# ViV99/slam-experiments

Measured on NVIDIA B200. Metric: hamming_pairs_per_sec, higher is better.
Workload: dtype u8

## Files before the change

### slam_experiments_b200/csrc/hm_tc.cu

```cuda
#include <math.h>
#include <stdlib.h>

#include <mutex>
#include <type_traits>

#include <cuda_fp16.h>

#include "hm_common.cuh"
#include "hm_tcgen05.cuh"

#ifndef HM_F4_TILE_N
#define HM_F4_TILE_N 128
#endif

namespace hm {

namespace {

constexpr int kRowBlock = 128;
constexpr int kMBlocks = 2;
constexpr int kBlockM = kRowBlock * kMBlocks;
constexpr int kSlabBytes = kRowBlock * 128;
constexpr int kPadRows = HM_PREPARED_TILE_ROWS;
constexpr int kTmemCols = 512;
constexpr uint32_t kSpinLimit = 1u << 26;

static_assert(kPadRows % kBlockM == 0, "prepared padding must cover whole query blocks");

struct CoreI8 {
    using Acc = int;
    static constexpr int kSlabs = 2;
    static constexpr int kRowBytes = HM_PREPARED_ROW_BYTES;
    static constexpr int kTileN = 128;
    static constexpr int kStages = 4;
    static constexpr int kUnits = 4;
    static constexpr int kColSplit = 1;
    static constexpr bool kRegisterHandover = false;
    static constexpr bool kScales = false;
    static constexpr int kPrologueTiles = 45;
    static __device__ __forceinline__ Acc lowest() { return INT_MIN; }
    static __device__ __forceinline__ Acc from_bits(uint32_t x) { return (int)x; }
    static __device__ __forceinline__ Acc max3(Acc a, Acc b, Acc c) { return __vimax3_s32(a, b, c); }
    static __device__ __forceinline__ Acc max2(Acc a, Acc b) { return max(a, b); }
    static __device__ __forceinline__ bool valid(Acc v) { return v >= -256; }
    static __device__ __forceinline__ unsigned distance(Acc v) { return (unsigned)((256 - v) >> 1); }
    static __device__ __forceinline__ unsigned encode(Acc v) { return (unsigned)(v + 257); }
    static __device__ __forceinline__ Acc floor_from(unsigned e) { return (int)e - 259; }
    static __device__ __forceinline__ uint32_t pack2(uint32_t lo, uint32_t hi) { return ((uint32_t)max((int)lo, -32768) & 0xFFFFu) | ((uint32_t)max((int)hi, -32768) << 16); }
    static __device__ __forceinline__ Acc unpack(uint32_t p, int hi) { return hi ? (int)p >> 16 : (int)(short)(p & 0xFFFFu); }
    static constexpr uint32_t kLowestBits = 0x80000000u;
};

struct CoreF4 {
    using Acc = float;
    static constexpr int kSlabs = 1;
    static constexpr int kRowBytes = HM_PREPARED_F4_ROW_BYTES;
    static constexpr int kTileN = HM_F4_TILE_N;
#ifndef HM_F4_STAGES
#define HM_F4_STAGES 6
#endif
    static constexpr int kStages = HM_F4_TILE_N == 96 ? 10 : HM_F4_TILE_N == 64 ? 14 : HM_F4_STAGES;
#ifndef HM_F4_UNITS
#define HM_F4_UNITS (HM_F4_TILE_N == 96 ? 5 : HM_F4_TILE_N == 64 ? 7 : 3)
#endif
    static constexpr int kUnits = HM_F4_UNITS;
    static constexpr int kColSplit = 2;
    static constexpr bool kRegisterHandover = true;
    static constexpr bool kScales = true;
    static constexpr int kPrologueTiles = 90;
    static __device__ __forceinline__ Acc lowest() { return -INFINITY; }
    static __device__ __forceinline__ Acc from_bits(uint32_t x) { return __uint_as_float(x); }
    static __device__ __forceinline__ Acc max3(Acc a, Acc b, Acc c) { return fmaxf(fmaxf(a, b), c); }
    static __device__ __forceinline__ Acc max2(Acc a, Acc b) { return fmaxf(a, b); }
    static __device__ __forceinline__ bool valid(Acc v) { return v >= -256.0f; }
    static __device__ __forceinline__ unsigned distance(Acc v) { return (unsigned)((256 - (int)v) >> 1); }
    static __device__ __forceinline__ unsigned encode(Acc v) { return (unsigned)((int)v + 257); }
    static __device__ __forceinline__ Acc floor_from(unsigned e) { return (float)((int)e - 259); }
    static __device__ __forceinline__ uint32_t pack2(uint32_t lo, uint32_t hi)
    {
        const __half2 h = __floats2half2_rn(__uint_as_float(lo), __uint_as_float(hi));
        return *reinterpret_cast<const uint32_t*>(&h);
    }
    static __device__ __forceinline__ Acc unpack(uint32_t p, int hi)
    {
        const __half2 h = *reinterpret_cast<const __half2*>(&p);
        return hi ? __high2float(h) : __low2float(h);
    }
    static constexpr uint32_t kLowestBits = 0xFF800000u;
};

template <class C> __host__ __device__ constexpr int row_block_bytes() { return kRowBlock * C::kRowBytes; }
template <class C> __host__ __device__ constexpr int a_bytes() { return kMBlocks * row_block_bytes<C>(); }
template <class C> __host__ __device__ constexpr int b_stage_bytes() { return C::kTileN * C::kRowBytes; }
template <class C> __host__ __device__ constexpr int epilogue_warps() { return 4 * kMBlocks * C::kColSplit; }
template <class C> __host__ __device__ constexpr int control_warps() { return C::kRegisterHandover ? 4 : 2; }
template <class C> __host__ __device__ constexpr int threads() { return 32 * (control_warps<C>() + epilogue_warps<C>()); }
constexpr int kHandoverBytes = kBlockM * 16;
constexpr int kBarrierBytes = 512;
template <class C> __host__ __device__ constexpr int smem_bytes() { return 1024 + a_bytes<C>() + C::kStages * b_stage_bytes<C>() + kBarrierBytes + kHandoverBytes; }
static_assert((2 * CoreF4::kStages + 1 + 2 * CoreF4::kUnits) * 8 + 16 <= kBarrierBytes, "barrier block");
static_assert((2 * CoreI8::kStages + 1 + 2 * CoreI8::kUnits) * 8 + 16 <= kBarrierBytes, "barrier block");
__host__ __device__ constexpr int ct_gcd(int a, int b) { return b == 0 ? a : ct_gcd(b, a % b); }
template <class C> __host__ __device__ constexpr int issuer_period() { return C::kStages / ct_gcd(C::kStages, C::kUnits) * C::kUnits; }
constexpr int kScaleCols = 32;
constexpr int kScaleCol = kTmemCols - kScaleCols;
static_assert(CoreF4::kUnits * CoreF4::kTileN <= kScaleCol, "accumulator units must end before the scale factors");

struct PrepareParams {
    const uint8_t* bits;
    long long n, stride, batch_stride;
    long long padded_rows;
    uint8_t* out;
};

__global__ void __launch_bounds__(256) hm_prepare_kernel(const PrepareParams P)
{
    const long long chunks_per_problem = P.padded_rows * 16;
    const long long o = (long long)blockIdx.x * blockDim.x + threadIdx.x;
    if (o >= chunks_per_problem) return;
    const int b = blockIdx.y;
    const long long rb = o >> 11;
    const int rem = (int)(o & 2047);
    const int slab = rem >> 10;
    const int rem2 = rem & 1023;
    const int rr = (rem2 >> 3) & 7;
    const int r = ((rem2 >> 6) << 3) | rr;
    const int c = (rem2 & 7) ^ rr;
    const long long row = rb * kRowBlock + r;
    uint4 v = make_uint4(0, 0, 0, 0);
    if (row < P.n) {
        const uint8_t* src = P.bits + (long long)b * P.batch_stride + row * P.stride + slab * 16 + c * 2;
        const unsigned bits16 = (unsigned)src[0] | ((unsigned)src[1] << 8);
        unsigned w[4];
#pragma unroll
        for (int i = 0; i < 4; ++i) {
            const unsigned nib = (bits16 >> (4 * i)) & 0xF;
            const unsigned spread = (nib & 1) | ((nib & 2) << 7) | ((nib & 4) << 14) | ((nib & 8) << 21);
            w[i] = (spread * 0xFEu) ^ 0xFFFFFFFFu;
        }
        v = make_uint4(w[0], w[1], w[2], w[3]);
    }
    uint4* dst = reinterpret_cast<uint4*>(P.out + (long long)b * P.padded_rows * HM_PREPARED_ROW_BYTES);
    dst[o] = v;
}

__device__ __forceinline__ uint4 expand_bits_e2m1(unsigned bits32)
{
    unsigned w[4];
#pragma unroll
    for (int i = 0; i < 4; ++i) {
        const unsigned by = (bits32 >> (8 * i)) & 0xFF;
        unsigned sgn = 0;
#pragma unroll
        for (int j = 0; j < 8; ++j) sgn |= ((by >> j) & 1u) << (4 * j + 3);
        w[i] = 0xAAAAAAAAu ^ sgn;
    }
    return make_uint4(w[0], w[1], w[2], w[3]);
}

__global__ void __launch_bounds__(256) hm_prepare_f4_kernel(const PrepareParams P)
{
    const long long chunks_per_problem = P.padded_rows * 8;
    const long long o = (long long)blockIdx.x * blockDim.x + threadIdx.x;
    if (o >= chunks_per_problem) return;
    const int b = blockIdx.y;
    const long long rb = o >> 10;
    const int rem = (int)(o & 1023);
    const int rr = (rem >> 3) & 7;
    const int r = ((rem >> 6) << 3) | rr;
    const int c = (rem & 7) ^ rr;
    const long long row = rb * kRowBlock + r;
    uint4 v = make_uint4(0, 0, 0, 0);
    if (row < P.n) {
        const unsigned bits32 = *reinterpret_cast<const unsigned*>(P.bits + (long long)b * P.batch_stride + row * P.stride + c * 4);
        v = expand_bits_e2m1(bits32);
    }
    uint4* dst = reinterpret_cast<uint4*>(P.out + (long long)b * P.padded_rows * HM_PREPARED_F4_ROW_BYTES);
    dst[o] = v;
}

struct TcParams {
    const uint8_t* qbits;
// ... 104 lines not shown
__device__ __forceinline__ void tmem_ld_fence4(uint32_t (&a)[32], uint32_t (&b)[32], uint32_t (&c)[32], uint32_t (&d)[32])
{
    asm volatile("tcgen05.wait::ld.sync.aligned;\n" : HM_R32(a), HM_R32(b), HM_R32(c), HM_R32(d) : : "memory");
}
__device__ __forceinline__ void tmem_ld_fence48(uint32_t (&a)[32], uint32_t (&b)[16])
{
    asm volatile("tcgen05.wait::ld.sync.aligned;\n" : HM_R32(a), HM_R8(b, 0), HM_R8(b, 8) : : "memory");
}
__device__ __forceinline__ void tmem_ld_fence64(uint32_t (&a)[64])
{
    asm volatile("tcgen05.wait::ld.sync.aligned;\n" : HM_R8(a, 0), HM_R8(a, 8), HM_R8(a, 16), HM_R8(a, 24), HM_R8(a, 32), HM_R8(a, 40), HM_R8(a, 48), HM_R8(a, 56) : : "memory");
}

template <class C, int kMode, int kGroups = 4>
__device__ __forceinline__ void scan_chunk(const uint32_t* r, unsigned colbase, Top2<typename C::Acc>& s)
{
    using Acc = typename C::Acc;
    static_assert(kGroups == 2 || kGroups == 4 || kGroups == 8, "8-column groups per compare");
    Acc gm[kGroups];
#pragma unroll
    for (int g = 0; g < kGroups; ++g) {
        const int o = g * 8;
        gm[g] = C::max3(C::max3(C::from_bits(r[o]), C::from_bits(r[o + 1]), C::from_bits(r[o + 2])),
                        C::max3(C::from_bits(r[o + 3]), C::from_bits(r[o + 4]), C::from_bits(r[o + 5])),
                        C::max2(C::from_bits(r[o + 6]), C::from_bits(r[o + 7])));
    }
    Acc m;
    if constexpr (kGroups == 8) m = C::max3(C::max3(gm[0], gm[1], gm[2]), C::max3(gm[3], gm[4], gm[5]), C::max2(gm[6], gm[7]));
    else if constexpr (kGroups == 4) m = C::max3(gm[0], gm[1], C::max2(gm[2], gm[3]));
    else m = C::max2(gm[0], gm[1]);
    constexpr bool kFloor = kMode == 1, kTop1 = kMode == 2;
    if (m > (kFloor ? s.f : kTop1 ? s.v1 : s.v2)) {
#if HM_TC_TRACE
        s.slow += 1;
#endif
#pragma unroll
        for (int g = 0; g < kGroups; ++g) {
            const Acc x = gm[g];
            if (x > (kFloor ? s.f : kTop1 ? s.v1 : s.v2)) {
                const int o = g * 8;
                const uint32_t p0 = C::pack2(r[o], r[o + 1]), p1 = C::pack2(r[o + 2], r[o + 3]);
                const uint32_t p2 = C::pack2(r[o + 4], r[o + 5]), p3 = C::pack2(r[o + 6], r[o + 7]);
                const unsigned idx = colbase + o;
                if (kTop1 || x > s.v1) {
                    if (!kTop1) {
                        s.v2 = s.v1; s.i2 = s.i1;
                        s.sb[0] = s.sa[0]; s.sb[1] = s.sa[1]; s.sb[2] = s.sa[2]; s.sb[3] = s.sa[3];
                    }
                    s.v1 = x; s.i1 = idx;
                    s.sa[0] = p0; s.sa[1] = p1; s.sa[2] = p2; s.sa[3] = p3;
                } else {
                    s.v2 = x; s.i2 = idx;
                    s.sb[0] = p0; s.sb[1] = p1; s.sb[2] = p2; s.sb[3] = p3;
                }
                if (kFloor) s.f = C::max2(s.v2, s.f);
            }
        }
    }
}

template <class C, int kN>
__device__ __forceinline__ void mask_tail(uint32_t* r, unsigned colbase, unsigned limit)
{
    if (colbase + kN > limit) {
#pragma unroll
        for (int j = 0; j < kN; ++j)
            if (colbase + j >= limit) r[j] = C::kLowestBits;
    }
}

#ifndef HM_ARRIVE_ELECT
#define HM_ARRIVE_ELECT 1
#endif
#ifndef HM_SCAN_FLAT64
#define HM_SCAN_FLAT64 1
#endif
#ifndef HM_FLOOR_DENSE_TILES
#define HM_FLOOR_DENSE_TILES 32
#endif
#ifndef HM_FLOOR_LATE_MASK
#define HM_FLOOR_LATE_MASK 15
#endif

#ifndef HM_F4_A_TMEM
#define HM_F4_A_TMEM 0
#endif
constexpr int kATmemCol = 384;
constexpr int kATmemColsPerBlock = 32;

template <class C>
__device__ __forceinline__ void issue_half(int h, uint32_t a_block, uint32_t b_stage, uint32_t tmem_d, uint32_t idesc,
                                           uint32_t tmem_sf)
{
    constexpr int kHalf = C::kSlabs * 2;
#pragma unroll
    for (int jj = 0; jj < kHalf; ++jj) {
        const int j = h * kHalf + jj;
        const int slab = j >> 2, k = j & 3;
        const uint64_t db = ptx::kmajor_sw128_desc_from_lo(b_stage + ((slab * kSlabBytes + k * 32) >> 4));
        if constexpr (C::kScales && HM_F4_A_TMEM) {
            ptx::mma_mxf4_ts(tmem_d, a_block + 8 * j, db, idesc, tmem_sf, tmem_sf + kScaleCols / 2, j != 0);
        } else {
            const uint64_t da = ptx::kmajor_sw128_desc_from_lo(a_block + ((slab * kSlabBytes + k * 32) >> 4));
            if constexpr (C::kScales) ptx::mma_mxf4_ss(tmem_d, da, db, idesc, tmem_sf, tmem_sf + kScaleCols / 2, j != 0);
            else                      ptx::mma_i8_ss(tmem_d, da, db, idesc, j != 0);
        }
    }
}

template <class C, int kMode>
__device__ __forceinline__ void tc_knn2_body(const TcParams& P)
{
    constexpr bool kFloor = kMode == 1;
    using Acc = typename C::Acc;
    constexpr int kStages = C::kStages;
    constexpr int kUnits = C::kUnits;
    constexpr int kABytes = a_bytes<C>();
    constexpr int kBStageBytes = b_stage_bytes<C>();
    constexpr int kRowBlockBytes = row_block_bytes<C>();
    constexpr int kTileN = C::kTileN;

    extern __shared__ uint8_t smem_raw[];
    uint8_t* smem = smem_raw + ((1024u - (ptx::smem_u32(smem_raw) & 1023u)) & 1023u);
    uint8_t* smem_a = smem;
    uint8_t* smem_b = smem + kABytes;
    uint64_t* bars = reinterpret_cast<uint64_t*>(smem + kABytes + kStages * kBStageBytes);
    uint64_t* full_bar = bars;
    uint64_t* empty_bar = bars + kStages;
    uint64_t* a_full_bar = bars + 2 * kStages;
    uint64_t* tmem_full_bar = bars + 2 * kStages + 1;
    uint64_t* tmem_empty_bar = tmem_full_bar + kUnits;
    uint32_t* tmem_base_slot = reinterpret_cast<uint32_t*>(tmem_empty_bar + kUnits);
    uint32_t* smem_base_slot = tmem_base_slot + 2;
    ulonglong2* handover = reinterpret_cast<ulonglong2*>(smem + kABytes + kStages * kBStageBytes + kBarrierBytes);

    const int warp = __shfl_sync(0xffffffffu, threadIdx.x >> 5, 0);
    const int lane = threadIdx.x & 31;
    if (threadIdx.x == 0) cta_mark(P, 0);
    if (threadIdx.x == 0 && (blockIdx.x | blockIdx.y | blockIdx.z) == 0 && P.clock_probe) {
        unsigned long long t;
        asm volatile("mov.u64 %0, %%globaltimer;" : "=l"(t));
        P.clock_probe[0] = (long long)t;
        P.clock_probe[1] = clock64();
    }
    const int qb = blockIdx.x;
    const int split = blockIdx.y;
    const int b = blockIdx.z;

    const uint32_t cs = ptx::cluster_nctarank();
    const uint32_t crank = ptx::cluster_ctarank();
    const uint16_t cmask = (uint16_t)((1u << cs) - 1);
    const bool has_a = qb < P.q_blocks_valid;
    auto rows_present = [&]() -> long long { return P.nq_dyn ? min((long long)__ldg(P.nq_dyn + b), P.nq) : P.nq; };
    if (P.nq_dyn && (long long)(qb - (int)crank) * kBlockM >= rows_present()) return;

    const int tile_begin = split * P.tiles_per_split;
    const int tile_end = min(tile_begin + P.tiles_per_split, P.ntiles);
    const int my_tiles = tile_end - tile_begin;

    constexpr int kProducerWarp = kIssuerLast ? epilogue_warps<C>() : 0;
    constexpr int kIssuerWarp = kIssuerLast ? epilogue_warps<C>() + 1 : 1;
    constexpr int kFirstEpiWarp = kIssuerLast ? 0 : 2;
    static_assert(kIssuerLast || !C::kRegisterHandover, "the control warps must form the last warpgroup");
    static_assert(!C::kRegisterHandover || (epilogue_warps<C>() == 16 && threads<C>() == 640),
                  "the register budget (4 x 32 + 16 x 112 = 20 x 96) assumes 20 warps launched at 96 registers");
    if (warp == kProducerWarp && lane == 0) {
        *smem_base_slot = ptx::smem_u32(smem);
        for (int i = 0; i < kStages; ++i) {
            ptx::mbar_init(&full_bar[i], 1);
            ptx::mbar_init(&empty_bar[i], cs);
        }
        ptx::mbar_init(a_full_bar, 1);
        for (int i = 0; i < kUnits; ++i) {
            ptx::mbar_init(&tmem_full_bar[i], 1);
            ptx::mbar_init(&tmem_empty_bar[i], 4 * C::kColSplit);
        }
        ptx::fence_barrier_init();
        ptx::fence_proxy_async();
    } else if (warp == kIssuerWarp) {
        ptx::tmem_alloc(tmem_base_slot, kTmemCols);
        ptx::tmem_relinquish();
    }
    ptx::tc_fence_before();
    if (cs > 1) ptx::cluster_sync();
    else __syncthreads();
    ptx::tc_fence_after();
    const uint32_t tmem_base = *tmem_base_slot;

    if constexpr (C::kScales) {
        if (warp >= kFirstEpiWarp && warp < kFirstEpiWarp + 4) {
            uint32_t ones[32];
#pragma unroll
            for (int i = 0; i < 32; ++i) ones[i] = 0x7F7F7F7Fu;
            const uint32_t taddr = tmem_base + ((uint32_t)((warp & 3) * 32) << 16) + kScaleCol;
            static_assert(kScaleCols == 32, "one x32 store per lane quarter");
            ptx::tmem_st_32x32(taddr, ones);
            ptx::tmem_st_wait();
        }
        if (HM_F4_A_TMEM) {
            static_assert(!HM_F4_A_TMEM || C::kUnits * C::kTileN <= kATmemCol, "accumulator units overlap the A operand");
            static_assert(!HM_F4_A_TMEM || kATmemCol + kMBlocks * kATmemColsPerBlock <= kScaleCol, "A operand overlaps the scale factors");
            if (warp >= kFirstEpiWarp && warp < kFirstEpiWarp + 4 * kMBlocks) {
                const int wq = warp & 3, wblk = ((warp - kFirstEpiWarp) >> 2) & 1;
                const int r = wq * 32 + lane;
                const long long qrow = (long long)qb * kBlockM + wblk * kRowBlock + r;
                uint32_t words[32];
#pragma unroll
                for (int i = 0; i < 32; ++i) words[i] = 0u;
                if (qrow < rows_present()) {
                    if (P.qbits) {
                        const int* qidx = P.q_index ? P.q_index + (long long)b * P.q_index_batch_stride : nullptr;
                        const long long srow = qidx ? (long long)__ldg(qidx + qrow) : qrow;
                        const uint4* src = reinterpret_cast<const uint4*>(P.qbits + (long long)b * P.q_bits_batch_stride + srow * P.q_bits_stride);
                        const uint4 lo = src[0], hi = src[1];
                        const unsigned bits[8] = {lo.x, lo.y, lo.z, lo.w, hi.x, hi.y, hi.z, hi.w};
#pragma unroll
                        for (int c = 0; c < 8; ++c) {
                            const uint4 v = expand_bits_e2m1(bits[c]);
                            words[4 * c] = v.x; words[4 * c + 1] = v.y; words[4 * c + 2] = v.z; words[4 * c + 3] = v.w;
                        }
                    } else if (has_a) {
                        const uint8_t* img = P.qprep + ((long long)b * P.q_padded + (long long)qb * kBlockM + wblk * kRowBlock) * C::kRowBytes;
                        const uint4* row = reinterpret_cast<const uint4*>(img + (r >> 3) * 1024 + (r & 7) * 128);
#pragma unroll
                        for (int c = 0; c < 8; ++c) {
                            const uint4 v = row[c ^ (r & 7)];
                            words[4 * c] = v.x; words[4 * c + 1] = v.y; words[4 * c + 2] = v.z; words[4 * c + 3] = v.w;
                        }
                    }
                }
                ptx::tmem_st_32x32(tmem_base + ((uint32_t)(wq * 32) << 16) + kATmemCol + wblk * kATmemColsPerBlock, words);
                ptx::tmem_st_wait();
            }
        } else if (P.qbits) {
            const uint8_t* qsrc = P.qbits + (long long)b * P.q_bits_batch_stride;
            const int* qidx = P.q_index ? P.q_index + (long long)b * P.q_index_batch_stride : nullptr;
            const long long nq_eff = rows_present();
            for (int o = threadIdx.x; o < kBlockM * 8; o += blockDim.x) {
                const int blk = o >> 10, rem = o & 1023;
                const int rr = (rem >> 3) & 7;
                const int r = ((rem >> 6) << 3) | rr;
                const int c = (rem & 7) ^ rr;
                const long long qrow = (long long)qb * kBlockM + blk * kRowBlock + r;
                uint4 v = make_uint4(0, 0, 0, 0);
                if (qrow < nq_eff) {
                    const long long srow = qidx ? (long long)__ldg(qidx + qrow) : qrow;
                    v = expand_bits_e2m1(*reinterpret_cast<const unsigned*>(qsrc + srow * P.q_bits_stride + c * 4));
                }
                reinterpret_cast<uint4*>(smem_a)[o] = v;
            }
            ptx::fence_proxy_async();
        }
        ptx::tc_fence_before();
        __syncthreads();
        ptx::tc_fence_after();
    }

    if (threadIdx.x == 0) cta_mark(P, 1);
    ulonglong2 my_keys = make_ulonglong2(kNoMatch, kNoMatch);
    long long my_row = -1;
    int my_row_in_cta = 0;

    auto run_producer = [&]() {
        if (lane == 0) {
            if (has_a && !P.qbits && !(C::kScales && HM_F4_A_TMEM)) {
                const uint8_t* qsrc = P.qprep + ((long long)b * P.q_padded + (long long)qb * kBlockM) * C::kRowBytes;
                ptx::mbar_arrive_expect_tx(a_full_bar, kABytes);
                ptx::bulk_g2s(smem_a, qsrc, kABytes, a_full_bar);
            }
            const uint8_t* tsrc = P.tprep + (long long)b * P.t_padded * C::kRowBytes;
            const uint32_t piece = kBStageBytes / cs;
            for (int i = 0; i < (HM_TC_EXPERIMENT >= 5 ? 0 : my_tiles); ++i) {
                const int stage = i % kStages;
                const uint32_t use = i / kStages;
#if HM_TC_EXPERIMENT < 4
                bounded_wait(&empty_bar[stage], (use & 1) ^ 1, P.error_flag);
#endif
                trace_mark(P, i, 0);
                ptx::mbar_arrive_expect_tx(&full_bar[stage], kBStageBytes);
                uint8_t* dst = smem_b + stage * kBStageBytes + crank * piece;
                const uint8_t* src = tsrc + (long long)(tile_begin + i) * kBStageBytes + crank * piece;
                if (cs > 1) ptx::bulk_g2s_multicast(dst, src, piece, &full_bar[stage], cmask);
                else        ptx::bulk_g2s(dst, src, piece, &full_bar[stage]);
            }
        }
    };
    auto run_issuer = [&]() {
        const bool leader = ptx::elect_one();
        const uint32_t idesc = C::kScales ? ptx::make_mxf4_idesc(kRowBlock, kTileN) : ptx::make_i8_idesc(kRowBlock, kTileN);
        constexpr bool kATmem = C::kScales && HM_F4_A_TMEM;
        const uint32_t a_addr = kATmem ? tmem_base + kATmemCol : ptx::smem_u32(smem_a) >> 4;
        constexpr uint32_t kABlockStep = kATmem ? (uint32_t)kATmemColsPerBlock : (uint32_t)(kRowBlockBytes >> 4);
        const uint32_t b_addr = ptx::smem_u32(smem_b) >> 4;
        const uint32_t tmem_sf = tmem_base + kScaleCol;
        if (has_a && !P.qbits && !(C::kScales && HM_F4_A_TMEM)) bounded_wait(a_full_bar, 0, P.error_flag);
        constexpr int kPeriod = issuer_period<C>();
        static_assert(kPeriod % kStages == 0 && (2 * kPeriod) % kUnits == 0 && ((2 * kPeriod / kUnits) & 1) == 0,
                      "unit parities must repeat with the period");
        uint32_t sphase = 0;
        bool ready0 = false;
        for (int base = 0; base < my_tiles; base += kPeriod) {
#pragma unroll
            for (int j = 0; j < kPeriod; ++j) {
                if (base + j < my_tiles) {
                    const int stage = j % kStages;
                    const uint32_t full_par = sphase ^ ((j / kStages) & 1);
                    const int unit_a = (2 * j) % kUnits, unit_b = (2 * j + 1) % kUnits;
                    const uint32_t par_a = (((2 * j) / kUnits) & 1) ^ 1, par_b = (((2 * j + 1) / kUnits) & 1) ^ 1;
                    const uint32_t b_stage = b_addr + stage * (kBStageBytes >> 4);
                    if (leader) trace_mark(P, base + j, 7);
                    if (!ready0) {
#if HM_TC_EXPERIMENT < 4
                        bounded_wait(&full_bar[stage], full_par, P.error_flag);
#endif
#if HM_TC_EXPERIMENT < 3
                        bounded_wait(&tmem_empty_bar[unit_a], par_a, P.error_flag);
#endif
                    }
                    if (leader) trace_mark(P, base + j, 1);
                    ptx::tc_fence_after();
                    if (leader) issue_half<C>(0, a_addr, b_stage, tmem_base + unit_a * kTileN, idesc, tmem_sf);
#if HM_TC_EXPERIMENT >= 3
                    const bool ready1 = true;
#else
                    const bool ready1 = __all_sync(0xffffffffu, ptx::mbar_test_wait(&tmem_empty_bar[unit_b], par_b));
#endif
                    if (leader) {
                        issue_half<C>(1, a_addr, b_stage, tmem_base + unit_a * kTileN, idesc, tmem_sf);
#if HM_TC_EXPERIMENT != 6 && HM_COMMIT_MODE == 0
                        ptx::tc_commit(&tmem_full_bar[unit_a]);
#endif
                    }
                    if (!ready1) bounded_wait(&tmem_empty_bar[unit_b], par_b, P.error_flag);
                    if (leader) trace_mark(P, base + j, 6);
                    ptx::tc_fence_after();
                    if (leader) issue_half<C>(0, a_addr + kABlockStep, b_stage, tmem_base + unit_b * kTileN, idesc, tmem_sf);
                    ready0 = false;
                    if (base + j + 1 < my_tiles) {
                        const int n = j + 1;
#if HM_TC_EXPERIMENT >= 4
                        ready0 = true;
#else
                        ready0 = __all_sync(0xffffffffu,
                                            ptx::mbar_test_wait(&full_bar[n % kStages], sphase ^ ((n / kStages) & 1))
#if HM_TC_EXPERIMENT < 3
                                            && ptx::mbar_test_wait(&tmem_empty_bar[(2 * n) % kUnits], (((2 * n) / kUnits) & 1) ^ 1)
#endif
                                            );
#endif
                    }
                    if (leader) {
                        issue_half<C>(1, a_addr + kABlockStep, b_stage, tmem_base + unit_b * kTileN, idesc, tmem_sf);
#if HM_TC_EXPERIMENT == 6 || HM_COMMIT_MODE == 1
                        ptx::tc_commit(&tmem_full_bar[unit_a]);
#endif
                        ptx::tc_commit(&tmem_full_bar[unit_b]);
                        if (cs > 1) ptx::tc_commit_multicast(&empty_bar[stage], cmask);
                        else        ptx::tc_commit(&empty_bar[stage]);
                    }
                }
            }
            sphase ^= (kPeriod / kStages) & 1;
        }
        __syncwarp();
    };
    auto run_epilogue = [&]() {
        constexpr int kCols = kTileN / C::kColSplit;
        const int quarter = warp & 3;
        const int mblk = ((warp - kFirstEpiWarp) >> 2) & 1;
        const int half = (warp - kFirstEpiWarp) >> 3;
        const int row_in_cta = mblk * kRowBlock + quarter * 32 + lane;
        const long long row = (long long)qb * kBlockM + row_in_cta;
        Top2<Acc> s;
        s.v1 = s.v2 = C::lowest();
        s.i1 = s.i2 = 0;
#pragma unroll
        for (int e = 0; e < 4; ++e) s.sa[e] = s.sb[e] = 0;
        s.f = C::floor_from(0);
#if HM_TC_TRACE
        s.slow = 0;
#endif
        unsigned floor_code = 0;
        const long long first_row = (long long)tile_begin * kTileN;
        const unsigned limit = (unsigned)min((long long)my_tiles * kTileN, P.nt - first_row);
        const uint32_t bars_addr = ptx::lds_volatile_u32(ptx::smem_u32(smem_base_slot)) + kABytes + kStages * kBStageBytes;
        const uint32_t unit_full_addr = bars_addr + (2 * kStages + 1) * 8;
        const uint32_t unit_empty_addr = unit_full_addr + kUnits * 8;
        int unit = mblk;
        uint32_t unit_use = 0;
        unsigned floor_pending = 0;
        auto refresh_floor = [&](int i) {
            if constexpr (kFloor) {
                if (i < HM_FLOOR_DENSE_TILES || (i & HM_FLOOR_LATE_MASK) == 0) {
                    floor_code = max(floor_code, floor_pending);
                    s.f = C::max2(s.f, C::floor_from(floor_code));
                    if (row < P.nq) {
                        unsigned* floor_ptr = P.row_floor + ((long long)b * P.nq + row);
                        const unsigned e = C::valid(s.v2) ? C::encode(s.v2) : 0u;
                        if (e > floor_code) { atomicMax(floor_ptr, e); floor_code = e; }
                        floor_pending = __ldcg(floor_ptr);
                    }
                }
            }
        };
        auto process_tile = [&](int i) {
            bounded_wait_addr(unit_full_addr + unit * 8, unit_use & 1, P.error_flag);
#if HM_TC_TRACE == 2
            if (warp == kFirstEpiWarp && lane == 0 && (i == 8 || i == 32 || i == 64 || i == 192)) cta_mark(P, i == 8 ? 5 : i == 32 ? 6 : i == 64 ? 7 : 8);
#endif
            if (warp == kFirstEpiWarp && lane == 0) trace_mark(P, i, 3);
            if (warp == kFirstEpiWarp + 7 && lane == 0) trace_mark(P, i, 5);
            ptx::tc_fence_after();
            const uint32_t taddr = tmem_base + ((uint32_t)(quarter * 32) << 16) + unit * kTileN + half * kCols;
            const unsigned colbase = (unsigned)i * kTileN + half * kCols;
            if constexpr (C::kColSplit == 1) {
                uint32_t r0[32], r1[32], r2[32], r3[32];
                ptx::tmem_ld_32x32(taddr, r0);
                ptx::tmem_ld_32x32(taddr + 32, r1);
                ptx::tmem_ld_32x32(taddr + 64, r2);
                ptx::tmem_ld_32x32(taddr + 96, r3);
                refresh_floor(i);
                tmem_ld_fence4(r0, r1, r2, r3);
                ptx::tc_fence_before();
                __syncwarp();
                if (HM_ARRIVE_ELECT ? ptx::elect_one() : lane == 0) ptx::mbar_arrive_addr(unit_empty_addr + unit * 8);
                if (colbase + kCols > limit) {
                    mask_tail<C, 32>(r0, colbase, limit);
                    mask_tail<C, 32>(r1, colbase + 32, limit);
                    mask_tail<C, 32>(r2, colbase + 64, limit);
                    mask_tail<C, 32>(r3, colbase + 96, limit);
                }
                scan_chunk<C, kMode>(r0, colbase, s);
                scan_chunk<C, kMode>(r1, colbase + 32, s);
                scan_chunk<C, kMode>(r2, colbase + 64, s);
                scan_chunk<C, kMode>(r3, colbase + 96, s);
            } else {
                if constexpr (kCols == 64) {
                    uint32_t r[64];
#if HM_TC_EXPERIMENT < 2
                    ptx::tmem_ld_32x64(taddr, r);
                    refresh_floor(i);
                    tmem_ld_fence64(r);
#endif
                    ptx::tc_fence_before();
                    __syncwarp();
                    if (HM_ARRIVE_ELECT ? ptx::elect_one() : lane == 0) ptx::mbar_arrive_addr(unit_empty_addr + unit * 8);
#if HM_TC_EXPERIMENT != 0
                    unit += 2;
                    if (unit >= kUnits) { unit -= kUnits; ++unit_use; }
                    return;
#endif
                    mask_tail<C, 64>(r, colbase, limit);
#if HM_SCAN_FLAT64
                    scan_chunk<C, kMode, 8>(r, colbase, s);
#else
                    scan_chunk<C, kMode>(r, colbase, s);
                    scan_chunk<C, kMode>(r + 32, colbase + 32, s);
#endif
                } else if constexpr (kCols == 32) {
                    uint32_t r[32];
                    ptx::tmem_ld_32x32(taddr, r);
                    refresh_floor(i);
                    asm volatile("tcgen05.wait::ld.sync.aligned;\n" : HM_R32(r) : : "memory");
                    ptx::tc_fence_before();
                    __syncwarp();
                    if (HM_ARRIVE_ELECT ? ptx::elect_one() : lane == 0) ptx::mbar_arrive_addr(unit_empty_addr + unit * 8);
                    mask_tail<C, 32>(r, colbase, limit);
                    scan_chunk<C, kMode>(r, colbase, s);
                } else {
                    static_assert(kCols == 64 || kCols == 48, "column split");
                    uint32_t r0[32], r1[16];
                    ptx::tmem_ld_32x32(taddr, r0);
                    ptx::tmem_ld_32x16(taddr + 32, r1);
                    refresh_floor(i);
                    tmem_ld_fence48(r0, r1);
                    ptx::tc_fence_before();
                    __syncwarp();
                    if (HM_ARRIVE_ELECT ? ptx::elect_one() : lane == 0) ptx::mbar_arrive_addr(unit_empty_addr + unit * 8);
                    mask_tail<C, 32>(r0, colbase, limit);
                    mask_tail<C, 16>(r1, colbase + 32, limit);
                    scan_chunk<C, kMode>(r0, colbase, s);
                    scan_chunk<C, kMode, 2>(r1, colbase + 32, s);
                }
            }
            unit += 2;
            if (unit >= kUnits) { unit -= kUnits; ++unit_use; }
            if (warp == kFirstEpiWarp && lane == 0) trace_mark(P, i, 4);
        };
#pragma unroll 1
        for (int i = 0; i < my_tiles; ++i) process_tile(i);
        if (warp == kFirstEpiWarp && lane == 0) cta_mark(P, 2);
#if HM_TC_TRACE
        if (P.trace) {
            const long long cta = ((long long)blockIdx.z * gridDim.y + blockIdx.y) * gridDim.x + blockIdx.x;
            long long* rec = P.trace + kTraceTiles * kTraceSlots + cta * kCtaSlots;
            const unsigned any = __reduce_max_sync(0xffffffffu, s.slow);
            const unsigned sum = __reduce_add_sync(0xffffffffu, s.slow);
            if (lane == 0) { atomicAdd((unsigned long long*)&rec[9], (unsigned long long)any); atomicAdd((unsigned long long*)&rec[10], (unsigned long long)sum); }
        }
#endif
        const unsigned long long gbase = P.train_base + (unsigned long long)first_row;
        auto fold_group = [&](Acc v, unsigned i0, const uint32_t (&p)[4]) {
            if (!C::valid(v)) return;
#pragma unroll
            for (int e = 0; e < 8; ++e) {
                const Acc x = C::unpack(p[e >> 1], e & 1);
                if (C::valid(x)) top2_insert(my_keys.x, my_keys.y, ((unsigned long long)C::distance(x) << 32) | (gbase + i0 + e));
            }
        };
        fold_group(s.v1, s.i1, s.sa);
        if (kMode != 2) fold_group(s.v2, s.i2, s.sb);
        else my_keys.y = kNoMatch;
        if (half == 1) handover[row_in_cta] = my_keys;
        else my_row = row;
        my_row_in_cta = row_in_cta;
    };

    auto run_tail = [&](auto worker_tag) {
        constexpr bool kWorker = decltype(worker_tag)::value;
        ptx::tc_fence_before();
        if (cs > 1) ptx::cluster_sync();
        else __syncthreads();
        if (kWorker && threadIdx.x == 0) cta_mark(P, 3);
        if (warp == kIssuerWarp) {
            ptx::tc_fence_after();
            ptx::tmem_dealloc(tmem_base, kTmemCols);
        }
        if (kWorker && my_row >= 0 && my_row < rows_present()) {
            if constexpr (C::kColSplit == 2) {
                const ulonglong2 o = handover[my_row_in_cta];
                top2_insert(my_keys.x, my_keys.y, o.x);
                top2_insert(my_keys.x, my_keys.y, o.y);
            }
            unsigned long long* out = P.out + (long long)split * P.out_split_stride + ((long long)b * P.nq + my_row) * 2;
            *reinterpret_cast<ulonglong2*>(out) = my_keys;
            if (!P.counters) select_candidate(P.sel, b, my_keys);
        }
        if (P.counters) {
            int* flag = reinterpret_cast<int*>(tmem_base_slot + 1);
            if (last_cta_arrives(&P.counters[(long long)b * gridDim.x + qb], (unsigned)P.splits, flag)) {
                const long long row = (long long)qb * kBlockM + threadIdx.x;
                const bool has_row = kWorker && threadIdx.x < kBlockM && row < rows_present();
                ulonglong2 k = make_ulonglong2(kNoMatch, kNoMatch);
                if (has_row) fold_partials(P.out, P.splits, P.out_split_stride, (long long)b * P.nq + row, k.x, k.y);
                if (P.xch.world > 1 && (long long)qb * kBlockM < P.nq) k = exchange_and_merge(P.xch, row, has_row, k, qb);
                if (has_row) {
                    *reinterpret_cast<ulonglong2*>(P.final_out + ((long long)b * P.nq + row) * 2) = k;
                    select_candidate(P.sel, b, k);
                }
            }
        }
        if (kWorker && threadIdx.x == 0) cta_mark(P, 4);
        if (kWorker && threadIdx.x == 0 && (blockIdx.x | blockIdx.y | blockIdx.z) == 0 && P.clock_probe) {
            unsigned long long t;
            asm volatile("mov.u64 %0, %%globaltimer;" : "=l"(t));
            P.clock_probe[2] = (long long)t;
            P.clock_probe[3] = clock64();
        }
    };

    if constexpr (C::kRegisterHandover) {
        if (warp >= kProducerWarp) {
            asm volatile("setmaxnreg.dec.sync.aligned.u32 32;\n");
            if (warp == kProducerWarp) run_producer();
            else if (warp == kIssuerWarp) run_issuer();
            run_tail(std::false_type{});
            return;
        }
        asm volatile("setmaxnreg.inc.sync.aligned.u32 112;\n");
        run_epilogue();
        run_tail(std::true_type{});
    } else {
        if (warp == kProducerWarp) run_producer();
        else if (warp == kIssuerWarp) run_issuer();
        else run_epilogue();
// ... 238 lines not shown
    P.ntiles = pl.ntiles;
    P.train_base = train_base;
    P.error_flag = static_cast<int*>(ws);
    P.clock_probe = reinterpret_cast<long long*>(static_cast<uint8_t*>(ws) + HM_WS_CLOCK_PROBE_OFFSET);
    P.q_blocks_valid = P.q_padded / kBlockM;
    const char* trace_path = getenv("HM_I8_TRACE");
    if (trace_path) {
        if (const char* tf = getenv("HM_TRACE_FIRST")) P.trace_first = atoi(tf);
        const size_t trace_words = (size_t)kTraceTiles * kTraceSlots + (size_t)pl.qblocks * pl.splits * batch * kCtaSlots;
        HM_CUDA_CHECK(cudaMalloc(&P.trace, sizeof(long long) * trace_words));
        HM_CUDA_CHECK(cudaMemset(P.trace, 0, sizeof(long long) * trace_words));
    }
    const long long rows = nq * batch;
    unsigned* counters = reinterpret_cast<unsigned*>(static_cast<uint8_t*>(ws) + 256);
    unsigned long long* partials = reinterpret_cast<unsigned long long*>(static_cast<uint8_t*>(ws) + 256 + cbytes);
    P.splits = pl.splits;
    if (pl.splits > 1 || keep_partials) {
        P.out = partials;
        P.out_split_stride = rows * 2;
    }
    const bool fused_exchange = exchange && exchange->world > 1;
    if (fused_exchange) {
        if (batch != 1 || keep_partials) {
            set_error("fused exchange needs batch == 1 and an output buffer");
            return HM_ERR_INVALID_ARGUMENT;
        }
        static_assert(kBlockM == kExchangeRows, "flag granularity = query block");
        P.xch = *exchange;
        P.out = partials;
        P.out_split_stride = rows * 2;
    }
    bool zero_block = false;
    const bool floor_eligible = !top1 && !P.nq_dyn && pl.tiles_per_split <= floor_max_tiles() &&
                                (pl.splits > 1 || (C::kColSplit > 1 && pl.ntiles >= floor_min_tiles_unsplit()));
    if (floor_eligible) {
        P.row_floor = reinterpret_cast<unsigned*>(reinterpret_cast<uint8_t*>(counters) + counters_bytes(pl.qblocks * batch));
        zero_block = true;
    }
    if ((pl.splits > 1 || fused_exchange) && !keep_partials) {
        P.counters = counters;
        P.final_out = out;
        zero_block = true;
    } else if (!(pl.splits > 1 || keep_partials)) {
        P.out = out;
        P.out_split_stride = 0;
    }
    static const bool keep_floors = getenv("HM_KEEP_FLOORS") != nullptr;
    if (zero_block) HM_CUDA_CHECK(cudaMemsetAsync(counters, 0, keep_floors ? counters_bytes(pl.qblocks * batch) : cbytes, stream));
    if (pl.qblocks > 0x7FFFFFFFll || pl.splits > 65535 || batch > 65535) {
        set_error("grid too large");
        return HM_ERR_UNSUPPORTED;
    }
    cudaLaunchConfig_t cfg{};
    cfg.gridDim = dim3((unsigned)pl.qblocks, (unsigned)pl.splits, (unsigned)batch);
    cfg.blockDim = dim3(threads<C>());
    cfg.dynamicSmemBytes = smem_bytes<C>();
    cfg.stream = stream;
    cudaLaunchAttribute attr[1];
    attr[0].id = cudaLaunchAttributeClusterDimension;
    attr[0].val.clusterDim.x = (unsigned)pl.cluster;
    attr[0].val.clusterDim.y = 1;
    attr[0].val.clusterDim.z = 1;
    cfg.attrs = attr;
    cfg.numAttrs = 1;
    profile_mark(true, stream);
    cudaError_t le = cudaLaunchKernelEx(&cfg, kernel_of<C>(P.row_floor ? 1 : top1 ? 2 : 0), P);
    profile_mark(false, stream);
    if (le != cudaSuccess) {
        set_error("cudaLaunchKernelEx(tensor-core k-NN kernel, cluster %d) failed: %s", pl.cluster, cudaGetErrorString(le));
        return HM_ERR_CUDA;
    }
    HM_CUDA_CHECK(cudaGetLastError());
    if (trace_path) {
        static long long host[kTraceTiles * kTraceSlots];
        HM_CUDA_CHECK(cudaStreamSynchronize(stream));
        HM_CUDA_CHECK(cudaMemcpy(host, P.trace, sizeof(host), cudaMemcpyDeviceToHost));
        {
            const size_t nctas = (size_t)pl.qblocks * pl.splits * batch;
            long long* rec = (long long*)malloc(nctas * kCtaSlots * sizeof(long long));
            if (rec && cudaMemcpy(rec, P.trace + kTraceTiles * kTraceSlots, nctas * kCtaSlots * sizeof(long long), cudaMemcpyDeviceToHost) == cudaSuccess) {
                char path[1024];
                snprintf(path, sizeof(path), "%s.ctas", trace_path);
                if (FILE* f = fopen(path, "w")) {
                    fprintf(f, "# cta entry_ns prologue_done loop_done final_barrier exit tile8 tile32 tile64 tile192 smid slow_warp_chunks_lb slow_lane_chunks (globaltimer ns since the first entry); grid=(%lld,%d,%d)\n", pl.qblocks, pl.splits, batch);
                    long long t0 = -1;
                    for (size_t c = 0; c < nctas; ++c) if (rec[c * kCtaSlots] && (t0 < 0 || rec[c * kCtaSlots] < t0)) t0 = rec[c * kCtaSlots];
                    for (size_t c = 0; c < nctas; ++c) {
                        fprintf(f, "%zu", c);
                        for (int k = 0; k < 9; ++k) fprintf(f, " %lld", rec[c * kCtaSlots + k] ? rec[c * kCtaSlots + k] - t0 : -1);
                        fprintf(f, " %lld %lld %lld", rec[c * kCtaSlots + 11], rec[c * kCtaSlots + 9], rec[c * kCtaSlots + 10]);
                        for (int k = 0; k < 9; ++k) fprintf(f, " %lld", rec[c * kCtaSlots + 12 + k] ? rec[c * kCtaSlots + 12 + k] - rec[c * kCtaSlots + 12] : -1);
                        fprintf(f, "\n");
                    }
                    fclose(f);
                }
            }
            free(rec);
        }
        cudaFree(P.trace);
        if (FILE* f = fopen(trace_path, "w")) {
            fprintf(f, "# tile producer_issue issuer_ready (unused) epi2_full epi2_scanned epi9_full issuer_unit1_free issuer_loop_top (cycles since first stamp); tiles/CTA=%d splits=%d cluster=%d core=%s\n",
                    pl.tiles_per_split, pl.splits, pl.cluster, C::kScales ? "mxf4" : "i8");
            long long t0 = host[0];
            for (int i = 0; i < kTraceTiles; ++i) {
                fprintf(f, "%d", i + P.trace_first);
                for (int k = 0; k < 8; ++k) fprintf(f, " %lld", host[i * kTraceSlots + k] ? host[i * kTraceSlots + k] - t0 : -1);
                fprintf(f, "\n");
            }
            fclose(f);
        }
    }
    if (keep_partials) {
        if (out_partials) *out_partials = partials;
        if (out_groups) *out_groups = pl.splits;
    }
    return HM_OK;
}

template <class C>
int launch_prepare_of(const uint8_t* bits, long long n, long long stride, long long batch_stride, int batch,
                      void* prepared, cudaStream_t stream)
{
    if (n <= 0 || batch <= 0) return HM_OK;
    PrepareParams P{};
    P.bits = bits; P.n = n; P.stride = stride; P.batch_stride = batch_stride;
    P.padded_rows = padded_rows<C>(n);
    P.out = static_cast<uint8_t*>(prepared);
    const long long chunks = P.padded_rows * (C::kRowBytes / 16);
    dim3 grid((unsigned)ceil_div(chunks, 256), (unsigned)batch);
    if (C::kScales) hm_prepare_f4_kernel<<<grid, 256, 0, stream>>>(P);
    else            hm_prepare_kernel<<<grid, 256, 0, stream>>>(P);
    HM_CUDA_CHECK(cudaGetLastError());
    return HM_OK;
}

template <class C>
int launch_knn2_of(const KnnProblem& p, unsigned long long* out, void* ws, size_t ws_bytes, int sm_count, cudaStream_t stream)
{
    const size_t need = workspace_bytes_of<C>(p.nq, p.nt, p.batch, sm_count, true);
    if (!ws || ws_bytes < need) {
        set_error("workspace too small: need %zu bytes, got %zu", need, ws_bytes);
        return HM_ERR_WORKSPACE;
    }
    const size_t head = workspace_bytes_of<C>(p.nq, p.nt, p.batch, sm_count, false);
    uint8_t* qprep = static_cast<uint8_t*>(ws) + head;
    uint8_t* tprep = qprep + (size_t)padded_rows<C>(p.nq) * C::kRowBytes * p.batch;
    int rc = HM_OK;
    QueryBits qb{};
    if (C::kScales) {
        qb.bits = p.q; qb.stride = p.q_stride; qb.batch_stride = p.q_batch_stride;
    } else {
        rc = launch_prepare_of<C>(p.q, p.nq, p.q_stride, p.q_batch_stride, p.batch, qprep, stream);
        if (rc != HM_OK) return rc;
    }
    rc = launch_prepare_of<C>(p.t, p.nt, p.t_stride, p.t_batch_stride, p.batch, tprep, stream);
    if (rc != HM_OK) return rc;
    if (p.select && !C::kScales) {
        set_error("candidate selection exists for the kind::mxf4 core only");
        return HM_ERR_UNSUPPORTED;
    }
    return launch_prepared<C>(qprep, p.nq, tprep, p.nt, p.batch, p.train_base, out, ws, head, sm_count, stream, nullptr,
                              nullptr, nullptr, p.top1, &qb, p.select);
}

}

size_t prepared_bytes(long long n, int variant)
{
    return variant == HM_VARIANT_F4 ? (size_t)padded_rows<CoreF4>(n) * CoreF4::kRowBytes : (size_t)padded_rows<CoreI8>(n) * CoreI8::kRowBytes;
}

int launch_prepare(const uint8_t* bits, long long n, long long stride, long long batch_stride, int batch,
                   void* prepared, int variant, cudaStream_t stream)
{
    return variant == HM_VARIANT_F4 ? launch_prepare_of<CoreF4>(bits, n, stride, batch_stride, batch, prepared, stream)
// ... 94 lines not shown
```

Baseline: 13860.

## Enable A operand in TMEM for MXF4 path and drop A from shared memory

Turns on by default the path where the query (A) operand of the MXF4 MMA lives in tensor memory, and removes the A buffer from the shared memory budget when that path is active. The epilogue's release of each accumulator unit now carries a fake data dependency on the loaded registers, so the barrier arrive cannot be hoisted ahead of the TMEM loads. It also adds a trace-only check that the A words stored in TMEM match the expected values. This cuts shared-memory traffic and footprint for the A operand, at the cost of using TMEM columns and relying on the tcgen05 A-from-TMEM MMA form being correct.

```diff
diff --git a/slam_experiments_b200/csrc/hm_tc.cu b/slam_experiments_b200/csrc/hm_tc.cu
--- a/slam_experiments_b200/csrc/hm_tc.cu
+++ b/slam_experiments_b200/csrc/hm_tc.cu
@@ -11,6 +11,10 @@
 
 #ifndef HM_F4_TILE_N
 #define HM_F4_TILE_N 128
+#endif
+
+#ifndef HM_F4_A_TMEM
+#define HM_F4_A_TMEM 1
 #endif
 
 namespace hm {
@@ -26,6 +30,9 @@
 constexpr uint32_t kSpinLimit = 1u << 26;
 
 static_assert(kPadRows % kBlockM == 0, "prepared padding must cover whole query blocks");
+constexpr bool kATmem = HM_F4_A_TMEM != 0;
+constexpr int kATmemCol = 384;
+constexpr int kATmemColsPerBlock = 32;
 
 struct CoreI8 {
     using Acc = int;
@@ -91,13 +98,14 @@
 
 template <class C> __host__ __device__ constexpr int row_block_bytes() { return kRowBlock * C::kRowBytes; }
 template <class C> __host__ __device__ constexpr int a_bytes() { return kMBlocks * row_block_bytes<C>(); }
+template <class C> __host__ __device__ constexpr int a_smem_bytes() { return C::kScales && kATmem ? 0 : a_bytes<C>(); }
 template <class C> __host__ __device__ constexpr int b_stage_bytes() { return C::kTileN * C::kRowBytes; }
 template <class C> __host__ __device__ constexpr int epilogue_warps() { return 4 * kMBlocks * C::kColSplit; }
 template <class C> __host__ __device__ constexpr int control_warps() { return C::kRegisterHandover ? 4 : 2; }
 template <class C> __host__ __device__ constexpr int threads() { return 32 * (control_warps<C>() + epilogue_warps<C>()); }
 constexpr int kHandoverBytes = kBlockM * 16;
 constexpr int kBarrierBytes = 512;
-template <class C> __host__ __device__ constexpr int smem_bytes() { return 1024 + a_bytes<C>() + C::kStages * b_stage_bytes<C>() + kBarrierBytes + kHandoverBytes; }
+template <class C> __host__ __device__ constexpr int smem_bytes() { return 1024 + a_smem_bytes<C>() + C::kStages * b_stage_bytes<C>() + kBarrierBytes + kHandoverBytes; }
 static_assert((2 * CoreF4::kStages + 1 + 2 * CoreF4::kUnits) * 8 + 16 <= kBarrierBytes, "barrier block");
 static_assert((2 * CoreI8::kStages + 1 + 2 * CoreI8::kUnits) * 8 + 16 <= kBarrierBytes, "barrier block");
 __host__ __device__ constexpr int ct_gcd(int a, int b) { return b == 0 ? a : ct_gcd(b, a % b); }
@@ -368,12 +376,6 @@
 #define HM_FLOOR_LATE_MASK 15
 #endif
 
-#ifndef HM_F4_A_TMEM
-#define HM_F4_A_TMEM 0
-#endif
-constexpr int kATmemCol = 384;
-constexpr int kATmemColsPerBlock = 32;
-
 template <class C>
 __device__ __forceinline__ void issue_half(int h, uint32_t a_block, uint32_t b_stage, uint32_t tmem_d, uint32_t idesc,
                                            uint32_t tmem_sf)
@@ -384,7 +386,7 @@
         const int j = h * kHalf + jj;
         const int slab = j >> 2, k = j & 3;
         const uint64_t db = ptx::kmajor_sw128_desc_from_lo(b_stage + ((slab * kSlabBytes + k * 32) >> 4));
-        if constexpr (C::kScales && HM_F4_A_TMEM) {
+        if constexpr (C::kScales && kATmem) {
             ptx::mma_mxf4_ts(tmem_d, a_block + 8 * j, db, idesc, tmem_sf, tmem_sf + kScaleCols / 2, j != 0);
         } else {
             const uint64_t da = ptx::kmajor_sw128_desc_from_lo(a_block + ((slab * kSlabBytes + k * 32) >> 4));
@@ -401,7 +403,8 @@
     using Acc = typename C::Acc;
     constexpr int kStages = C::kStages;
     constexpr int kUnits = C::kUnits;
-    constexpr int kABytes = a_bytes<C>();
+    constexpr bool kATmemA = C::kScales && kATmem;
+    constexpr int kABytes = a_smem_bytes<C>();
     constexpr int kBStageBytes = b_stage_bytes<C>();
     constexpr int kRowBlockBytes = row_block_bytes<C>();
     constexpr int kTileN = C::kTileN;
@@ -473,6 +476,32 @@
     ptx::tc_fence_after();
     const uint32_t tmem_base = *tmem_base_slot;
 
+    auto a_row_words = [&](int wblk, int r, uint32_t (&words)[32]) {
+#pragma unroll
+        for (int i = 0; i < 32; ++i) words[i] = 0u;
+        const long long qrow = (long long)qb * kBlockM + wblk * kRowBlock + r;
+        if (qrow >= rows_present()) return;
+        if (P.qbits) {
+            const int* qidx = P.q_index ? P.q_index + (long long)b * P.q_index_batch_stride : nullptr;
+            const long long srow = qidx ? (long long)__ldg(qidx + qrow) : qrow;
+            const uint4* src = reinterpret_cast<const uint4*>(P.qbits + (long long)b * P.q_bits_batch_stride + srow * P.q_bits_stride);
+            const uint4 lo = src[0], hi = src[1];
+            const unsigned bits[8] = {lo.x, lo.y, lo.z, lo.w, hi.x, hi.y, hi.z, hi.w};
+#pragma unroll
+            for (int c = 0; c < 8; ++c) {
+                const uint4 v = expand_bits_e2m1(bits[c]);
+                words[4 * c] = v.x; words[4 * c + 1] = v.y; words[4 * c + 2] = v.z; words[4 * c + 3] = v.w;
+            }
+        } else if (has_a) {
+            const uint8_t* img = P.qprep + ((long long)b * P.q_padded + (long long)qb * kBlockM + wblk * kRowBlock) * C::kRowBytes;
+            const uint4* row = reinterpret_cast<const uint4*>(img + (r >> 3) * 1024 + (r & 7) * 128);
+#pragma unroll
+            for (int c = 0; c < 8; ++c) {
+                const uint4 v = row[c ^ (r & 7)];
+                words[4 * c] = v.x; words[4 * c + 1] = v.y; words[4 * c + 2] = v.z; words[4 * c + 3] = v.w;
+            }
+        }
+    };
     if constexpr (C::kScales) {
         if (warp >= kFirstEpiWarp && warp < kFirstEpiWarp + 4) {
             uint32_t ones[32];
@@ -483,38 +512,13 @@
             ptx::tmem_st_32x32(taddr, ones);
             ptx::tmem_st_wait();
         }
-        if (HM_F4_A_TMEM) {
-            static_assert(!HM_F4_A_TMEM || C::kUnits * C::kTileN <= kATmemCol, "accumulator units overlap the A operand");
-            static_assert(!HM_F4_A_TMEM || kATmemCol + kMBlocks * kATmemColsPerBlock <= kScaleCol, "A operand overlaps the scale factors");
+        if (kATmemA) {
+            static_assert(!kATmemA || C::kUnits * C::kTileN <= kATmemCol, "accumulator units overlap the A operand");
+            static_assert(!kATmemA || kATmemCol + kMBlocks * kATmemColsPerBlock <= kScaleCol, "A operand overlaps the scale factors");
             if (warp >= kFirstEpiWarp && warp < kFirstEpiWarp + 4 * kMBlocks) {
                 const int wq = warp & 3, wblk = ((warp - kFirstEpiWarp) >> 2) & 1;
-                const int r = wq * 32 + lane;
-                const long long qrow = (long long)qb * kBlockM + wblk * kRowBlock + r;
                 uint32_t words[32];
-#pragma unroll
-                for (int i = 0; i < 32; ++i) words[i] = 0u;
-                if (qrow < rows_present()) {
-                    if (P.qbits) {
-                        const int* qidx = P.q_index ? P.q_index + (long long)b * P.q_index_batch_stride : nullptr;
-                        const long long srow = qidx ? (long long)__ldg(qidx + qrow) : qrow;
-                        const uint4* src = reinterpret_cast<const uint4*>(P.qbits + (long long)b * P.q_bits_batch_stride + srow * P.q_bits_stride);
-                        const uint4 lo = src[0], hi = src[1];
-                        const unsigned bits[8] = {lo.x, lo.y, lo.z, lo.w, hi.x, hi.y, hi.z, hi.w};
-#pragma unroll
-                        for (int c = 0; c < 8; ++c) {
-                            const uint4 v = expand_bits_e2m1(bits[c]);
-                            words[4 * c] = v.x; words[4 * c + 1] = v.y; words[4 * c + 2] = v.z; words[4 * c + 3] = v.w;
-                        }
-                    } else if (has_a) {
-                        const uint8_t* img = P.qprep + ((long long)b * P.q_padded + (long long)qb * kBlockM + wblk * kRowBlock) * C::kRowBytes;
-                        const uint4* row = reinterpret_cast<const uint4*>(img + (r >> 3) * 1024 + (r & 7) * 128);
-#pragma unroll
-                        for (int c = 0; c < 8; ++c) {
-                            const uint4 v = row[c ^ (r & 7)];
-                            words[4 * c] = v.x; words[4 * c + 1] = v.y; words[4 * c + 2] = v.z; words[4 * c + 3] = v.w;
-                        }
-                    }
-                }
+                a_row_words(wblk, wq * 32 + lane, words);
                 ptx::tmem_st_32x32(tmem_base + ((uint32_t)(wq * 32) << 16) + kATmemCol + wblk * kATmemColsPerBlock, words);
                 ptx::tmem_st_wait();
             }
@@ -549,7 +553,7 @@
 
     auto run_producer = [&]() {
         if (lane == 0) {
-            if (has_a && !P.qbits && !(C::kScales && HM_F4_A_TMEM)) {
+            if (has_a && !P.qbits && !kATmemA) {
                 const uint8_t* qsrc = P.qprep + ((long long)b * P.q_padded + (long long)qb * kBlockM) * C::kRowBytes;
                 ptx::mbar_arrive_expect_tx(a_full_bar, kABytes);
                 ptx::bulk_g2s(smem_a, qsrc, kABytes, a_full_bar);
@@ -574,12 +578,11 @@
     auto run_issuer = [&]() {
         const bool leader = ptx::elect_one();
         const uint32_t idesc = C::kScales ? ptx::make_mxf4_idesc(kRowBlock, kTileN) : ptx::make_i8_idesc(kRowBlock, kTileN);
-        constexpr bool kATmem = C::kScales && HM_F4_A_TMEM;
-        const uint32_t a_addr = kATmem ? tmem_base + kATmemCol : ptx::smem_u32(smem_a) >> 4;
-        constexpr uint32_t kABlockStep = kATmem ? (uint32_t)kATmemColsPerBlock : (uint32_t)(kRowBlockBytes >> 4);
+        const uint32_t a_addr = kATmemA ? tmem_base + kATmemCol : ptx::smem_u32(smem_a) >> 4;
+        constexpr uint32_t kABlockStep = kATmemA ? (uint32_t)kATmemColsPerBlock : (uint32_t)(kRowBlockBytes >> 4);
         const uint32_t b_addr = ptx::smem_u32(smem_b) >> 4;
         const uint32_t tmem_sf = tmem_base + kScaleCol;
-        if (has_a && !P.qbits && !(C::kScales && HM_F4_A_TMEM)) bounded_wait(a_full_bar, 0, P.error_flag);
+        if (has_a && !P.qbits && !kATmemA) bounded_wait(a_full_bar, 0, P.error_flag);
         constexpr int kPeriod = issuer_period<C>();
         static_assert(kPeriod % kStages == 0 && (2 * kPeriod) % kUnits == 0 && ((2 * kPeriod / kUnits) & 1) == 0,
                       "unit parities must repeat with the period");
@@ -674,6 +677,16 @@
         const uint32_t unit_empty_addr = unit_full_addr + kUnits * 8;
         int unit = mblk;
         uint32_t unit_use = 0;
+        const uint32_t opaque_zero = bars_addr - (ptx::smem_u32(smem) + kABytes + kStages * kBStageBytes);
+        auto release_unit = [&](uint32_t last) {
+            ptx::tc_fence_before();
+            __syncwarp();
+            if (HM_ARRIVE_ELECT ? ptx::elect_one() : lane == 0) ptx::mbar_arrive_addr(unit_empty_addr + unit * 8 + (last & opaque_zero));
+        };
+        auto next_unit = [&]() {
+            unit += 2;
+            if (unit >= kUnits) { unit -= kUnits; ++unit_use; }
+        };
         unsigned floor_pending = 0;
         auto refresh_floor = [&](int i) {
             if constexpr (kFloor) {
@@ -707,9 +720,7 @@
                 ptx::tmem_ld_32x32(taddr + 96, r3);
                 refresh_floor(i);
                 tmem_ld_fence4(r0, r1, r2, r3);
-                ptx::tc_fence_before();
-                __syncwarp();
-                if (HM_ARRIVE_ELECT ? ptx::elect_one() : lane == 0) ptx::mbar_arrive_addr(unit_empty_addr + unit * 8);
+                release_unit(r0[31] | r1[31] | r2[31] | r3[31]);
                 if (colbase + kCols > limit) {
                     mask_tail<C, 32>(r0, colbase, limit);
                     mask_tail<C, 32>(r1, colbase + 32, limit);
@@ -727,13 +738,12 @@
                     ptx::tmem_ld_32x64(taddr, r);
                     refresh_floor(i);
                     tmem_ld_fence64(r);
-#endif
-                    ptx::tc_fence_before();
-                    __syncwarp();
-                    if (HM_ARRIVE_ELECT ? ptx::elect_one() : lane == 0) ptx::mbar_arrive_addr(unit_empty_addr + unit * 8);
+                    release_unit(r[63]);
+#else
+                    release_unit(0);
+#endif
 #if HM_TC_EXPERIMENT != 0
-                    unit += 2;
-                    if (unit >= kUnits) { unit -= kUnits; ++unit_use; }
+                    next_unit();
                     return;
 #endif
                     mask_tail<C, 64>(r, colbase, limit);
@@ -748,9 +758,7 @@
                     ptx::tmem_ld_32x32(taddr, r);
                     refresh_floor(i);
                     asm volatile("tcgen05.wait::ld.sync.aligned;\n" : HM_R32(r) : : "memory");
-                    ptx::tc_fence_before();
-                    __syncwarp();
-                    if (HM_ARRIVE_ELECT ? ptx::elect_one() : lane == 0) ptx::mbar_arrive_addr(unit_empty_addr + unit * 8);
+                    release_unit(r[31]);
                     mask_tail<C, 32>(r, colbase, limit);
                     scan_chunk<C, kMode>(r, colbase, s);
                 } else {
@@ -760,23 +768,39 @@
                     ptx::tmem_ld_32x16(taddr + 32, r1);
                     refresh_floor(i);
                     tmem_ld_fence48(r0, r1);
-                    ptx::tc_fence_before();
-                    __syncwarp();
-                    if (HM_ARRIVE_ELECT ? ptx::elect_one() : lane == 0) ptx::mbar_arrive_addr(unit_empty_addr + unit * 8);
+                    release_unit(r0[31] | r1[15]);
                     mask_tail<C, 32>(r0, colbase, limit);
                     mask_tail<C, 16>(r1, colbase + 32, limit);
                     scan_chunk<C, kMode>(r0, colbase, s);
                     scan_chunk<C, kMode, 2>(r1, colbase + 32, s);
                 }
             }
-            unit += 2;
-            if (unit >= kUnits) { unit -= kUnits; ++unit_use; }
+            next_unit();
             if (warp == kFirstEpiWarp && lane == 0) trace_mark(P, i, 4);
         };
 #pragma unroll 1
         for (int i = 0; i < my_tiles; ++i) process_tile(i);
         if (warp == kFirstEpiWarp && lane == 0) cta_mark(P, 2);
 #if HM_TC_TRACE
+        if (kATmemA && P.trace && half == 0) {
+            const long long cta = ((long long)blockIdx.z * gridDim.y + blockIdx.y) * gridDim.x + blockIdx.x;
+            long long* rec = P.trace + kTraceTiles * kTraceSlots + cta * kCtaSlots;
+            uint32_t got[32], want[32];
+            ptx::tmem_ld_32x32(tmem_base + ((uint32_t)(quarter * 32) << 16) + kATmemCol + mblk * kATmemColsPerBlock, got);
+            asm volatile("tcgen05.wait::ld.sync.aligned;\n" : HM_R32(got) : : "memory");
+            a_row_words(mblk, quarter * 32 + lane, want);
+            unsigned bad = 0;
+            for (int c = 0; c < 32; ++c) {
+                if (got[c] != want[c]) {
+                    if (bad == 0) {
+                        atomicMax((unsigned long long*)&rec[22], (unsigned long long)((row_in_cta << 8) | c) + 1);
+                        atomicExch((unsigned long long*)&rec[23], (unsigned long long)(got[c] ^ want[c]));
+                    }
+                    ++bad;
+                }
+            }
+            if (bad) atomicAdd((unsigned long long*)&rec[21], (unsigned long long)bad);
+        }
         if (P.trace) {
             const long long cta = ((long long)blockIdx.z * gridDim.y + blockIdx.y) * gridDim.x + blockIdx.x;
             long long* rec = P.trace + kTraceTiles * kTraceSlots + cta * kCtaSlots;
@@ -1181,7 +1205,7 @@
                 char path[1024];
                 snprintf(path, sizeof(path), "%s.ctas", trace_path);
                 if (FILE* f = fopen(path, "w")) {
-                    fprintf(f, "# cta entry_ns prologue_done loop_done final_barrier exit tile8 tile32 tile64 tile192 smid slow_warp_chunks_lb slow_lane_chunks (globaltimer ns since the first entry); grid=(%lld,%d,%d)\n", pl.qblocks, pl.splits, batch);
+                    fprintf(f, "# cta entry_ns prologue_done loop_done final_barrier exit tile8 tile32 tile64 tile192 smid slow_warp_chunks_lb slow_lane_chunks (globaltimer ns since the first entry), then the same nine as clock64 cycles, then A-in-TMEM check: bad_words first_bad (row<<8|col)+1 xor; grid=(%lld,%d,%d)\n", pl.qblocks, pl.splits, batch);
                     long long t0 = -1;
                     for (size_t c = 0; c < nctas; ++c) if (rec[c * kCtaSlots] && (t0 < 0 || rec[c * kCtaSlots] < t0)) t0 = rec[c * kCtaSlots];
                     for (size_t c = 0; c < nctas; ++c) {
@@ -1189,7 +1213,7 @@
                         for (int k = 0; k < 9; ++k) fprintf(f, " %lld", rec[c * kCtaSlots + k] ? rec[c * kCtaSlots + k] - t0 : -1);
                         fprintf(f, " %lld %lld %lld", rec[c * kCtaSlots + 11], rec[c * kCtaSlots + 9], rec[c * kCtaSlots + 10]);
                         for (int k = 0; k < 9; ++k) fprintf(f, " %lld", rec[c * kCtaSlots + 12 + k] ? rec[c * kCtaSlots + 12 + k] - rec[c * kCtaSlots + 12] : -1);
-                        fprintf(f, "\n");
+                        fprintf(f, " %lld %lld %lld\n", rec[c * kCtaSlots + 21], rec[c * kCtaSlots + 22], rec[c * kCtaSlots + 23]);
                     }
                     fclose(f);
                 }
```

Result: faster. 14660 (median of 6 runs) (+5.7%).
